# Farmadupe/vid_dup_finder_lib

Measured on AMD Instinct MI355X. Metric: hash-pairs/sec all-pairs Hamming (search(), tolerance 0.35) [+ frames/sec DCT-hash in 'summary.hash_summary'], higher is better.
Workload: dtype fp4 e2m1 ({0,1}) x fp4 -> f32 accumulate (exact half-integers < 2^11)

## Files before the change

vid_dup_finder_lib_amd/csrc/api.cpp:

```cpp
#include <algorithm>
#include <chrono>
#include <cmath>
#include <cstdio>
#include <cstdlib>
#include <cstring>
#include <memory>
#include <numeric>

#include "host_sort.h"
#include "vdf_ctx.h"
#include "window_class_layout.h"

namespace {
thread_local std::string g_create_error;
inline double now_ms() { return std::chrono::duration<double, std::milli>(std::chrono::steady_clock::now().time_since_epoch()).count(); }
}

vdf_ctx::~vdf_ctx()
{
    if (!subs.empty() || !workers.empty()) vdf_impl::destroy_multi(this);
    if (copy_pool) vdf_impl::destroy_copy_pool(this);
    for (auto &kv : axis_tables) {
        kv.second->start.release(); kv.second->size.release(); kv.second->w.release();
        delete kv.second;
    }
    for (auto &kv : mfma_tables) {
        kv.second->operand.release(); kv.second->bias.release(); kv.second->meta.release();
        delete kv.second;
    }
    for (auto &kv : box_tables) {
        kv.second->blob.release(); kv.second->entries.release();
        delete kv.second;
    }
    DevBuf *all[] = {&row_lo, &row_hi, &tile_lo, &tile_hi, &tile_first, &tile_count, &tile_offset, &counters,
                     &hits, &perm, &matched, &exp_cols, &exp_rows, &pop_cols, &pop_rows, &cand, &group_cmin, &group_offset, &group_blocks, &up_hashes,
                     &up_dur, &up_ref_hashes, &up_ref_dur, &small, &frames, &frames2, &out_hashes, &out_hashes2, &out_dc,
                     &out_dc2, &cos_table, &crops, &crop_desc, &crop_tables, &crop_desc2, &crop_tables2, &crop_work, &sort_scratch, &sort_scratch_pub, &hits2, &hit_bitmaps, &bitmap_gather,
                     &out_zero, &out_zero2, &up_zero, &variant_hashes, &align_plan, &align_scratch, &align_up, &seed_bitmap, &seed_plan, &seed_out, &seed_classes};
    for (DevBuf *b : all) b->release();
    for (PinBuf &b : pin) b.release();
    for (PinBuf &b : pin_out) b.release();
    pin_small.release();
    pin_ctrl.release();
    pin_crops.release();
    pin_desc.release();
    host_hits.buf.release();
    if (ev0) (void)hipEventDestroy(ev0);
    if (ev1) (void)hipEventDestroy(ev1);
    if (ev_mid) (void)hipEventDestroy(ev_mid);
    if (ev_wait) (void)hipEventDestroy(ev_wait);
    for (hipEvent_t e : ev_copy) if (e) (void)hipEventDestroy(e);
    for (hipEvent_t e : ev_done) if (e) (void)hipEventDestroy(e);
    if (copy_stream) (void)hipStreamDestroy(copy_stream);
    if (stream) (void)hipStreamDestroy(stream);
}

namespace vdf_impl {

void set_create_error(const std::string &msg) { g_create_error = msg; }

int fail(vdf_ctx *ctx, int code, const std::string &msg)
{
    if (ctx) ctx->err = msg;
    return code;
}

int fail_hip(vdf_ctx *ctx, hipError_t e, const char *what)
{
    std::string msg = std::string(what) + ": " + hipGetErrorString(e);
    (void)hipGetLastError();
    return fail(ctx, e == hipErrorOutOfMemory ? VDF_E_OOM : VDF_E_HIP, msg);
}

bool is_sorted_u32(const uint32_t *d, size_t n)
{
    for (size_t i = 1; i < n; i++)
        if (d[i] < d[i - 1]) return false;
    return true;
}

constexpr size_t kPinSmallBytes = 4u << 20;
constexpr uint64_t kDeviceSortHits = 1u << 17;
constexpr uint32_t kRefsMinWorkgroups = 2048;
constexpr uint64_t kSpecSortHits = 1u << 14;
constexpr uint64_t kFilterHits = 1u << 16;

int search_core(vdf_ctx *ctx, int mode, const uint64_t *d_col_hashes, const uint32_t *d_col_dur, size_t n_cols,
                const uint64_t *d_row_hashes, const uint32_t *d_row_dur, const uint32_t *d_row_perm, size_t n_rows,
                uint32_t tol_int, uint32_t shard_index, uint32_t shard_count, uint32_t row_begin, uint32_t row_end,
                const uint32_t *d_matched, uint32_t row_index_base, vdf_hit *hits, uint64_t capacity,
                uint64_t *n_hits_out, uint32_t *overflow_row_out, hipStream_t stream, bool replay_only, vdf_ctx::HostHits *staging,
                ShardExchange *fx)
{
    *n_hits_out = 0;
    *overflow_row_out = 0xFFFFFFFFu;
    if (n_rows == 0 || n_cols == 0) return VDF_OK;
    if (n_rows >= 0xFFFFFFFFull || n_cols >= 0xFFFFFFFFull) return fail(ctx, VDF_E_INVAL, "more than 2^32-1 hashes");
    if (shard_count == 0 || shard_index >= shard_count) return fail(ctx, VDF_E_INVAL, "bad shard index/count");
    VDF_HIP(ctx, hipSetDevice(ctx->device));
    const double t_enter = now_ms();

    vdf::SearchLaunch L{};
    const bool mfma = ctx->search_backend == 1;
    L.tile_rows = mfma ? (mode == 1 ? ctx->mfma_refs_rows : ctx->mfma_self_rows) : ctx->tile_rows;
    L.chunk_cols = mfma ? ctx->mfma_chunk_cols : ctx->chunk_cols;
    L.n_row_tiles = (uint32_t)((n_rows + L.tile_rows - 1) / L.tile_rows);
    if (mfma && L.chunk_cols == 0) {
        L.chunk_cols = 65536;
        while (L.chunk_cols > 4096 && (uint64_t)L.n_row_tiles * ((n_cols + L.chunk_cols - 1) / L.chunk_cols) < ctx->mfma_min_wgs) L.chunk_cols /= 2;
    }
    while ((uint64_t)L.n_row_tiles * ((n_cols + L.chunk_cols - 1) / L.chunk_cols) >= 0x40000000ull && L.chunk_cols < (1u << 22))
        L.chunk_cols *= 2;
    const size_t padded_rows = (size_t)L.n_row_tiles * L.tile_rows;
    VDF_HIP(ctx, ctx->row_lo.reserve(padded_rows * 4));
    VDF_HIP(ctx, ctx->row_hi.reserve(padded_rows * 4));
    VDF_HIP(ctx, ctx->tile_lo.reserve((size_t)L.n_row_tiles * 4));
    VDF_HIP(ctx, ctx->tile_hi.reserve((size_t)L.n_row_tiles * 4));
    VDF_HIP(ctx, ctx->tile_first.reserve((size_t)L.n_row_tiles * 4));
    VDF_HIP(ctx, ctx->tile_count.reserve((size_t)L.n_row_tiles * 4));
    VDF_HIP(ctx, ctx->tile_offset.reserve(((size_t)L.n_row_tiles + 1) * 4));
    VDF_HIP(ctx, ctx->counters.reserve(64));
    const uint64_t dev_cap = std::max<uint64_t>(capacity, 1);
    VDF_HIP(ctx, ctx->hits.reserve(dev_cap * sizeof(vdf_hit)));

    L.row_hashes = reinterpret_cast<const uint32_t *>(d_row_hashes);
    L.row_perm = d_row_perm;
    L.n_rows = (uint32_t)n_rows;
    L.row_index_base = row_index_base;
    L.col_hashes = reinterpret_cast<const uint32_t *>(d_col_hashes);
    L.n_cols = (uint32_t)n_cols;
    L.row_lo = ctx->row_lo.as<uint32_t>();
    L.row_hi = ctx->row_hi.as<uint32_t>();
    L.tile_lo = ctx->tile_lo.as<uint32_t>();
    L.tile_hi = ctx->tile_hi.as<uint32_t>();
    L.tile_first = ctx->tile_first.as<uint32_t>();
    L.tile_count = ctx->tile_count.as<uint32_t>();
    L.tile_offset = ctx->tile_offset.as<uint32_t>();
    L.tol = tol_int;
    L.matched = d_matched;
    L.self_mode = (mode == 0);
    L.shard_index = shard_index;
    L.shard_count = shard_count;
    L.hits = ctx->hits.as<vdf_hit>();
    L.capacity = capacity;
    L.counters = ctx->counters.as<unsigned long long>();
    L.overflow_row = reinterpret_cast<uint32_t *>(ctx->counters.as<unsigned long long>() + 4);

    L.prune_step = 16;
    if (ctx->mfma_prune_step >= 0) {
        L.prune_step = ctx->mfma_prune_step;
    } else {
        for (int st = 6; st <= 14; st++) {
            const double bits = 64.0 * (st + 1);
            if (bits / 2 - 2.0 * std::sqrt(bits) >= (double)tol_int + 1) { L.prune_step = st; break; }
        }
    }
    if (mfma) L.prune_step = L.prune_step <= 6 ? 6 : L.prune_step <= 8 ? 8 : L.prune_step <= 10 ? 10 : L.prune_step <= 14 ? L.prune_step : 16;
    else L.prune_step = L.prune_step <= 6 ? 6 : L.prune_step <= 10 ? 10 : L.prune_step <= 12 ? 12 : 16;
    if (mfma) {
        L.group_size = std::min<uint32_t>(ctx->mfma_group, L.n_row_tiles);
        L.n_groups = (L.n_row_tiles + L.group_size - 1) / L.group_size;
        if (L.n_groups > 1024) return fail(ctx, VDF_E_INVAL, "too many row-tile groups");
        VDF_HIP(ctx, ctx->group_cmin.reserve((size_t)L.n_groups * 4));
        VDF_HIP(ctx, ctx->group_offset.reserve(((size_t)L.n_groups + 1) * 4));
        VDF_HIP(ctx, ctx->group_blocks.reserve((size_t)L.n_groups * 4));
        L.group_blocks = ctx->group_blocks.as<uint32_t>();
        L.group_cmin = ctx->group_cmin.as<uint32_t>();
        L.group_offset = ctx->group_offset.as<uint32_t>();
        const uint32_t k_steps = (uint32_t)(L.prune_step < 15 ? L.prune_step + 1 : 16);
        const uint32_t col_pad = (uint32_t)((n_cols + vdf::kMfmaRowPad - 1) / vdf::kMfmaRowPad * vdf::kMfmaRowPad) + vdf::kMfmaColPad;
        VDF_HIP(ctx, ctx->exp_cols.reserve((size_t)col_pad * 512));
        VDF_HIP(ctx, ctx->pop_cols.reserve((size_t)col_pad * 12));
        const ExpOwner want_owner{d_col_hashes, n_cols, k_steps, ctx->exp_cols.p};
        const bool reuse = ctx->pinned_db == d_col_hashes && ctx->pinned_n == n_cols && ctx->exp_owner == want_owner;
        if (!reuse) {
            ctx->exp_owner = ExpOwner{};
            VDF_HIP(ctx, vdf::launch_expand_fp4(L.col_hashes, (uint32_t)n_cols, col_pad, ctx->exp_cols.p, k_steps,
                                                ctx->pop_cols.as<float>(), stream));
            ctx->exp_owner = want_owner;
        }
        L.col_exp = ctx->exp_cols.p;
        L.col_pop3 = ctx->pop_cols.as<float>();
        L.col_pad = col_pad;
        if (d_row_hashes == d_col_hashes) {
            L.row_exp = ctx->exp_cols.p;
            L.row_pop3 = L.col_pop3;
            L.row_pad = col_pad;
        } else {
            const uint32_t row_pad = (uint32_t)((padded_rows + 127) / 128 * 128);
            VDF_HIP(ctx, ctx->exp_rows.reserve((size_t)row_pad * 512));
            VDF_HIP(ctx, ctx->pop_rows.reserve((size_t)row_pad * 12));
            VDF_HIP(ctx, vdf::launch_expand_fp4(L.row_hashes, (uint32_t)n_rows, row_pad, ctx->exp_rows.p, k_steps,
                                                ctx->pop_rows.as<float>(), stream));
            L.row_exp = ctx->exp_rows.p;
            L.row_pop3 = ctx->pop_rows.as<float>();
            L.row_pad = row_pad;
        }
    }
    const unsigned long long init[8] = {0, 0, 0, 0, 0xFFFFFFFFull, 0, 0, 0};
    const bool pin_ok = ctx->pin_small.reserve(kPinSmallBytes) && ctx->pin_small.pinned;
    uint64_t spec = std::min<uint64_t>(capacity, std::max<uint64_t>(ctx->hits_guess + ctx->hits_guess / 4 + 1024, 8192));
    if (!pin_ok || spec * sizeof(vdf_hit) > kPinSmallBytes) spec = 0;
    const bool spec_sort = spec && ctx->hits_guess >= kSpecSortHits;
    if (spec_sort) VDF_HIP(ctx, hipMemsetAsync(ctx->hits.p, 0xFF, (size_t)spec * sizeof(vdf_hit), stream));
    const bool adapt_refs = mode == 1 && mfma && ctx->mfma_chunk_cols == 0;
    if (adapt_refs && ctx->refs_hint_cols == n_cols && ctx->refs_hint_rows == n_rows && ctx->refs_hint_chunk) L.chunk_cols = ctx->refs_hint_chunk;
    if (!ctx->pin_ctrl.reserve(256)) return fail(ctx, VDF_E_OOM, "pinned staging");
    unsigned long long *pre = ctx->pin_ctrl.as<unsigned long long>() + 8;
    uint32_t total_tiles = 0;
    unsigned long long unsorted = 0, admitted = 0;
    for (int pass = 0;; pass++) {
        VDF_HIP(ctx, hipMemcpyAsync(ctx->counters.p, init, sizeof init, hipMemcpyHostToDevice, stream));
        VDF_HIP(ctx, vdf::launch_windows_tiles(mode, d_col_dur, (uint32_t)n_cols, d_row_dur, d_row_perm, (uint32_t)n_rows,
                                               row_begin, row_end, shard_index, shard_count, L, stream));
        VDF_HIP(ctx, hipMemcpyAsync(pre, L.counters, 64, hipMemcpyDeviceToHost, stream));
        VDF_HIP(ctx, hipMemcpyAsync(pre + 8, mfma ? L.group_offset + L.n_groups : L.tile_offset + L.n_row_tiles, 4,
                                    hipMemcpyDeviceToHost, stream));
        VDF_HIP(ctx, hipMemcpyAsync(pre + 9, L.tile_offset + L.n_row_tiles, 4, hipMemcpyDeviceToHost, stream));
        VDF_HIP(ctx, hipStreamSynchronize(stream));
        total_tiles = *reinterpret_cast<const uint32_t *>(pre + 8);
        const uint32_t busy_tiles = *reinterpret_cast<const uint32_t *>(pre + 9);
        unsorted = pre[5];
        admitted = pre[2];
        if (!adapt_refs || pass > 0 || unsorted || busy_tiles == 0 || busy_tiles >= kRefsMinWorkgroups || L.chunk_cols <= 4096) break;
        uint64_t est = busy_tiles;
        while (L.chunk_cols > 4096 && est < kRefsMinWorkgroups) { L.chunk_cols /= 2; est *= 2; }
    }
    if (adapt_refs) { ctx->refs_hint_cols = n_cols; ctx->refs_hint_rows = n_rows; ctx->refs_hint_chunk = L.chunk_cols; }
    if (unsorted) return fail(ctx, VDF_E_INVAL, "durations are not ascending: pass the arrays in Search::sort order");
    if (total_tiles >= 0x7FFFFFFFu) return fail(ctx, VDF_E_INVAL, "tile count exceeds the grid limit");
    if (mfma) {
        const uint64_t want = ((uint64_t)((double)admitted * 6e-6) + (uint64_t)total_tiles * 8 * 8 + std::max<uint64_t>(capacity, 1ull << 20)) * ctx->cand_scale;
        L.cand_capacity = (uint32_t)std::min<uint64_t>(want, 0x40000000ull);
        if (ctx->cand_capacity_override)
            L.cand_capacity = (uint32_t)std::min<uint64_t>((uint64_t)ctx->cand_capacity_override * ctx->cand_scale, 0x40000000ull);
        const void *before = ctx->cand.p;
        VDF_HIP(ctx, ctx->cand.reserve((size_t)L.cand_capacity * 16));
        if (ctx->cand.p != before) ctx->cand_dirty = SIZE_MAX;
        const size_t slots = ctx->cand.cap / 16;
        const size_t fill = (ctx->cand_dirty == SIZE_MAX ? slots : std::min<size_t>(slots, ctx->cand_dirty)) * 16;
        if (fill) VDF_HIP(ctx, hipMemsetAsync(ctx->cand.p, 0xFF, fill, stream));
        ctx->cand_dirty = L.cand_capacity;
        L.cand = ctx->cand.p;
        L.cand_head = ctx->counters.as<unsigned long long>() + 6;
    }

    ctx->timing.prep_ms += (float)(now_ms() - t_enter);
    VDF_HIP(ctx, hipEventRecord(ctx->ev0, stream));
    if (mfma) {
        VDF_HIP(ctx, vdf::launch_hamming_tiles_mfma2(L, total_tiles, stream));
        VDF_HIP(ctx, hipEventRecord(ctx->ev_mid, stream));
        if (total_tiles) VDF_HIP(ctx, vdf::launch_resolve_candidates(L, stream));
    } else {
        VDF_HIP(ctx, vdf::launch_hamming_tiles(L, total_tiles, stream));
        VDF_HIP(ctx, hipEventRecord(ctx->ev_mid, stream));
    }
    VDF_HIP(ctx, hipEventRecord(ctx->ev1, stream));
    if (!ctx->pin_ctrl.reserve(256)) return fail(ctx, VDF_E_OOM, "pinned staging");
    unsigned long long *fin = ctx->pin_ctrl.as<unsigned long long>();
    VDF_HIP(ctx, hipMemcpyAsync(fin, ctx->counters.p, 64, hipMemcpyDeviceToHost, stream));
    unsigned row_bits = 1;
    while (row_bits < 32 && ((uint64_t)row_index_base + n_rows) >> row_bits) row_bits++;
    unsigned col_bits = 1;
    while (col_bits < 32 && ((uint64_t)n_cols >> col_bits)) col_bits++;
    if (spec_sort) {
        VDF_HIP(ctx, ctx->sort_scratch.reserve(vdf::sort_hits_scratch_bytes((size_t)spec)));
        VDF_HIP(ctx, vdf::launch_sort_hits(ctx->hits.as<vdf_hit>(), (size_t)spec, row_bits, ctx->sort_scratch.p, ctx->sort_scratch.cap, stream, col_bits));
    }
    if (spec) VDF_HIP(ctx, hipMemcpyAsync(ctx->pin_small.p, ctx->hits.p, (size_t)spec * sizeof(vdf_hit), hipMemcpyDeviceToHost, stream));
    VDF_HIP(ctx, hipStreamSynchronize(stream));
    const double t_synced = now_ms();
    float ms = 0.f, ms_stream = 0.f;
    VDF_HIP(ctx, hipEventElapsedTime(&ms, ctx->ev0, ctx->ev1));
// ... 3799 lines not shown
```

vid_dup_finder_lib_amd/csrc/hamming.hip:

```cpp
#include <algorithm>

#include "vdf_internal.h"

namespace vdf {

constexpr uint32_t kMaxBlocksPerLaunch = 4u << 20;

typedef const __attribute__((address_space(4))) uint32_t *const_u32_ptr;

__device__ __forceinline__ uint32_t sat_u32(double x)
{
    if (!(x == x)) return 0u;
    if (x <= 0.0) return 0u;
    if (x >= 4294967295.0) return 0xFFFFFFFFu;
    return (uint32_t)x;
}

__device__ __forceinline__ uint32_t partition_point_lt(const uint32_t *__restrict__ d, uint32_t n, uint32_t v)
{
    uint32_t lo = 0, hi = n;
    while (lo < hi) {
        uint32_t mid = lo + ((hi - lo) >> 1);
        if (d[mid] < v) lo = mid + 1; else hi = mid;
    }
    return lo;
}
__device__ __forceinline__ uint32_t partition_point_le(const uint32_t *__restrict__ d, uint32_t n, uint32_t v)
{
    uint32_t lo = 0, hi = n;
    while (lo < hi) {
        uint32_t mid = lo + ((hi - lo) >> 1);
        if (d[mid] <= v) lo = mid + 1; else hi = mid;
    }
    return lo;
}

__device__ __forceinline__ uint32_t wave_min(uint32_t v)
{
#pragma unroll
    for (int o = 32; o > 0; o >>= 1) v = min(v, (uint32_t)__shfl_xor((int)v, o, 64));
    return v;
}
__device__ __forceinline__ uint32_t wave_max(uint32_t v)
{
#pragma unroll
    for (int o = 32; o > 0; o >>= 1) v = max(v, (uint32_t)__shfl_xor((int)v, o, 64));
    return v;
}

__device__ __forceinline__ void wave_append_hits(bool hit, uint32_t row, uint32_t col, vdf_hit *__restrict__ hits,
                                                 unsigned long long capacity, unsigned long long *__restrict__ counters,
                                                 uint32_t *__restrict__ overflow_row)
{
    const unsigned long long bal = __builtin_amdgcn_ballot_w64(hit);
    if (bal == 0ull) return;
    const int leader = __builtin_ctzll(bal);
    unsigned long long base = 0;
    if ((int)(threadIdx.x & 63) == leader) base = atomicAdd(&counters[0], (unsigned long long)__builtin_popcountll(bal));
    base = ((unsigned long long)(uint32_t)__shfl((int)(base >> 32), leader, 64) << 32) | (uint32_t)__shfl((int)(uint32_t)base, leader, 64);
    if (hit) {
        const unsigned long long at = base + __builtin_amdgcn_mbcnt_hi((uint32_t)(bal >> 32), __builtin_amdgcn_mbcnt_lo((uint32_t)bal, 0u));
        if (at < capacity) {
            vdf_hit hp; hp.row = row; hp.col = col;
            hits[at] = hp;
        } else {
            atomicMin(overflow_row, row);
        }
    }
}

__global__ __launch_bounds__(256) void windows_tiles_kernel(
    int mode, const uint32_t *__restrict__ col_dur, uint32_t n_cols, const uint32_t *__restrict__ row_dur,
    const uint32_t *__restrict__ row_perm, uint32_t n_rows, uint32_t row_begin, uint32_t row_end, uint32_t shard_index,
    uint32_t shard_count, uint32_t tile_rows, uint32_t chunk_cols, uint32_t *__restrict__ row_lo,
    uint32_t *__restrict__ row_hi, uint32_t *__restrict__ tile_lo, uint32_t *__restrict__ tile_hi,
    uint32_t *__restrict__ tile_first, uint32_t *__restrict__ tile_count, unsigned long long *__restrict__ counters)
{
    __shared__ uint32_t s_min[4], s_max[4];
    __shared__ unsigned long long s_pairs[4];
    const uint32_t t = blockIdx.x;
    const bool mine = (t % shard_count) == shard_index;
    uint32_t mn = 0xFFFFFFFFu, mx = 0u;
    unsigned long long pairs = 0;
    for (uint32_t q = threadIdx.x; q < tile_rows; q += 256) {
// ... 156 lines not shown
#pragma unroll
            for (int q = 0; q < 8; q++) {
                const uint4 v = rp[q];
                rw[k][4 * q + 0] = v.x; rw[k][4 * q + 1] = v.y; rw[k][4 * q + 2] = v.z; rw[k][4 * q + 3] = v.w;
            }
            if (self_mode && matched && ((matched[src >> 5] >> (src & 31)) & 1u)) { lo = 0; hi = 0; }
        } else {
#pragma unroll
            for (int q = 0; q < 32; q++) rw[k][q] = 0u;
            lo = 0; hi = 0;
        }
        rlo[k] = lo; rhi[k] = hi; rid[k] = row_index_base + src;
    }

    const_u32_ptr cols = (const_u32_ptr)(uintptr_t)col_hashes;
    uint32_t n_early = 0;
    for (uint32_t c = c_begin; c < c_end; ++c) {
        const_u32_ptr cp = cols + (size_t)c * 32;
        uint32_t d[R];
#pragma unroll
        for (int k = 0; k < R; k++) d[k] = 0u;
#pragma unroll
        for (int w = 0; w < (CHKW < 32 ? CHKW : 32); ++w) {
            const uint32_t cw = cp[w];
#pragma unroll
            for (int k = 0; k < R; k++) d[k] += __builtin_popcount(rw[k][w] ^ cw);
        }
        uint32_t m = d[0];
#pragma unroll
        for (int k = 1; k < R; k++) m = min(m, d[k]);
        if (CHKW < 32) {
            if (__builtin_amdgcn_ballot_w64(m <= tol) == 0ull) { n_early += 1; continue; }
#pragma unroll
            for (int w = CHKW; w < 32; ++w) {
                const uint32_t cw = cp[w];
#pragma unroll
                for (int k = 0; k < R; k++) d[k] += __builtin_popcount(rw[k][w] ^ cw);
            }
            m = d[0];
#pragma unroll
            for (int k = 1; k < R; k++) m = min(m, d[k]);
        }
        if (__builtin_amdgcn_ballot_w64(m <= tol) != 0ull) {
            bool col_ok = true;
            if (matched) col_ok = ((((const_u32_ptr)(uintptr_t)matched)[c >> 5] >> (c & 31)) & 1u) == 0u;
            if (col_ok) {
#pragma unroll
                for (int k = 0; k < R; k++)
                    wave_append_hits(d[k] <= tol && c >= rlo[k] && c < rhi[k], rid[k], c, hits, capacity, counters, overflow_row);
            }
        }
    }
    if (threadIdx.x == 0) atomicAdd(&counters[1], (unsigned long long)(c_end - c_begin) * TILE_ROWS);
    if (CHKW < 32 && lane == 0 && n_early) atomicAdd(&counters[3], (unsigned long long)n_early * (64u * R));
}

typedef int v8i __attribute__((ext_vector_type(8)));
typedef int v4i __attribute__((ext_vector_type(4)));
typedef float v16f __attribute__((ext_vector_type(16)));

__global__ __launch_bounds__(256) void expand_fp4_kernel(const uint32_t *__restrict__ packed, uint32_t n,
                                                        uint32_t n_pad, uint4 *__restrict__ expanded,
                                                        uint32_t k_steps, float *__restrict__ pop,
                                                        float *__restrict__ popk, float *__restrict__ popkT)
{
    for (size_t idx = (size_t)blockIdx.x * 256 + threadIdx.x; idx < (size_t)n_pad * 32;
         idx += (size_t)gridDim.x * 256) {
    const uint32_t hsh = (uint32_t)(idx >> 5), dw = (uint32_t)idx & 31u;
    uint4 out = {0u, 0u, 0u, 0u};
    uint32_t w = 0;
    if (hsh < n) {
        w = packed[idx];
        uint32_t o[4];
#pragma unroll
        for (int j = 0; j < 4; j++) {
            uint32_t x = (w >> (8 * j)) & 0xFFu;
            x = (x | (x << 12)) & 0x000F000Fu;
            x = (x | (x << 6)) & 0x03030303u;
            x = (x | (x << 3)) & 0x11111111u;
            o[j] = x << 1;
        }
        out = make_uint4(o[0], o[1], o[2], o[3]);
    }
    expanded[idx] = out;
    if (pop) {
        uint32_t pc = (uint32_t)__builtin_popcount(w), pk = (dw & 15u) < k_steps ? pc : 0u;
#pragma unroll
        for (int o = 16; o > 0; o >>= 1) { pc += (uint32_t)__shfl_xor((int)pc, o, 32); pk += (uint32_t)__shfl_xor((int)pk, o, 32); }
        if (dw == 0) {
            pop[hsh] = (float)pc;
            popk[hsh] = (float)pk;
            popkT[(size_t)(hsh >> 7) * 128 + (hsh & 31u) * 4 + ((hsh >> 5) & 3u)] = (float)pk;
        }
    }
    }
}

template <int N>
struct IntC { static constexpr int value = N; };
template <int I, int N, class F>
__device__ __forceinline__ void static_for(F &&f)
{
    if constexpr (I < N) {
        f(IntC<I>{});
        static_for<I + 1, N>(f);
    }
}

constexpr uint32_t rowterm_row_of_lane(uint32_t l) { return (l & 3u) + 8u * ((l & 15u) >> 2) + 4u * (l >> 5); }
constexpr bool rowterm_map_matches_c_layout()
{
    for (uint32_t g = 0; g < 2; g++)
        for (uint32_t half = 0; half < 2; half++)
            for (uint32_t r = 0; r < 16; r++)
                if (rowterm_row_of_lane(32u * g + 16u * half + r) != (r & 3u) + 8u * (r >> 2) + 4u * g) return false;
    return true;
}
static_assert(rowterm_map_matches_c_layout(), "row-term lanes do not match the MFMA C layout");

struct CandEntry {
    uint32_t row_base;
    uint32_t col;
    uint32_t mask;
    uint32_t pad;
};

__global__ __launch_bounds__(256) void resolve_candidates_kernel(
    const CandEntry *__restrict__ cand, const unsigned long long *__restrict__ cand_head, uint32_t cand_capacity,
    const uint32_t *__restrict__ row_hashes, const uint32_t *__restrict__ row_perm, uint32_t n_rows, uint32_t row_index_base,
    const uint32_t *__restrict__ col_hashes, uint32_t n_cols, const uint32_t *__restrict__ row_lo,
    const uint32_t *__restrict__ row_hi, uint32_t tol, const uint32_t *__restrict__ matched, int self_mode,
    vdf_hit *__restrict__ hits, unsigned long long capacity, unsigned long long *__restrict__ counters,
    uint32_t *__restrict__ overflow_row)
{
    const uint32_t n = (uint32_t)min(*cand_head, (unsigned long long)cand_capacity);
    const uint32_t lane = threadIdx.x & 63, wave = threadIdx.x >> 6;
    constexpr uint32_t kStage = 512;
    __shared__ vdf_hit s_stage[4][kStage];
    uint32_t staged = 0;
    auto flush = [&]() {
        if (staged == 0) return;
        __builtin_amdgcn_fence(__ATOMIC_ACQ_REL, "wavefront");
        __builtin_amdgcn_wave_barrier();
        unsigned long long base = 0;
        if (lane == 0) base = atomicAdd(&counters[0], (unsigned long long)staged);
        base = ((unsigned long long)(uint32_t)__builtin_amdgcn_readfirstlane((int)(base >> 32)) << 32) |
               (uint32_t)__builtin_amdgcn_readfirstlane((int)(uint32_t)base);
        for (uint32_t k = lane; k < staged; k += 64) {
            const vdf_hit hp = s_stage[wave][k];
            if (base + k < capacity) hits[base + k] = hp;
            else atomicMin(overflow_row, hp.row);
        }
        __builtin_amdgcn_fence(__ATOMIC_ACQ_REL, "wavefront");
        __builtin_amdgcn_wave_barrier();
        staged = 0;
    };
    for (uint32_t e0 = blockIdx.x * 256 + (threadIdx.x & ~63u); e0 < n; e0 += gridDim.x * 256) {
        const uint32_t e = e0 + lane;
        CandEntry ce;
        ce.row_base = 0xFFFFFFFFu; ce.col = 0; ce.mask = 0; ce.pad = 0;
        if (e < n) ce = cand[e];
        uint32_t m = ce.mask;
        if (ce.row_base == 0xFFFFFFFFu || ce.col >= n_cols) m = 0;
        if (m && matched && ((matched[ce.col >> 5] >> (ce.col & 31)) & 1u)) m = 0;
        uint4 cw[8];
        if (m) {
            const uint4 *cp = reinterpret_cast<const uint4 *>(col_hashes + (size_t)ce.col * 32);
#pragma unroll
            for (int q = 0; q < 8; q++) cw[q] = cp[q];
        }
        while (__builtin_amdgcn_ballot_w64(m != 0u) != 0ull) {
            bool hit = false;
            uint32_t src = 0;
            if (m) {
                const uint32_t r = (uint32_t)__builtin_ctz(m);
                m &= m - 1;
                const uint32_t p = ce.row_base + (r & 3) + 8 * (r >> 2);
                if (p < n_rows) {
                    const uint32_t lo = row_lo[p], hi = row_hi[p];
                    if (ce.col >= lo && ce.col < hi) {
                        src = row_perm ? row_perm[p] : p;
                        if (!(self_mode && matched && ((matched[src >> 5] >> (src & 31)) & 1u))) {
                            const uint4 *rp = reinterpret_cast<const uint4 *>(row_hashes + (size_t)src * 32);
                            uint32_t d = 0;
#pragma unroll
                            for (int q = 0; q < 8; q++) {
                                const uint4 v = rp[q];
                                d += __builtin_popcount(v.x ^ cw[q].x) + __builtin_popcount(v.y ^ cw[q].y) +
                                     __builtin_popcount(v.z ^ cw[q].z) + __builtin_popcount(v.w ^ cw[q].w);
                            }
                            hit = d <= tol;
                        }
                    }
                }
            }
            const unsigned long long bal = __builtin_amdgcn_ballot_w64(hit);
            if (bal == 0ull) continue;
            const uint32_t cnt = (uint32_t)__builtin_popcountll(bal);
            if (staged + cnt > kStage) flush();
            if (hit) {
                vdf_hit hp; hp.row = row_index_base + src; hp.col = ce.col;
                s_stage[wave][staged + __builtin_amdgcn_mbcnt_hi((uint32_t)(bal >> 32), __builtin_amdgcn_mbcnt_lo((uint32_t)bal, 0u))] = hp;
            }
            staged += cnt;
        }
    }
    flush();
}

template <int CHK, int WAVES>
__global__ __launch_bounds__(64 * WAVES, 2) void hamming_mfma2_kernel(
    const uint4 *__restrict__ row_exp, const uint32_t *__restrict__ row_perm, uint32_t n_rows,
    uint32_t row_index_base, const uint4 *__restrict__ col_exp, const uint32_t *__restrict__ row_lo,
    const uint32_t *__restrict__ row_hi, const uint32_t *__restrict__ tile_lo, const uint32_t *__restrict__ tile_hi,
    const uint32_t *__restrict__ tile_first, const uint32_t *__restrict__ tile_count,
    const uint32_t *__restrict__ group_offset, const uint32_t *__restrict__ group_cmin, uint32_t n_groups,
    uint32_t group_size, uint32_t shard_index, uint32_t shard_count, uint32_t n_row_tiles, uint32_t chunk_cols,
    uint32_t tol, const uint32_t *__restrict__ matched, int self_mode, vdf_hit *__restrict__ hits,
    unsigned long long capacity, unsigned long long *__restrict__ counters, uint32_t *__restrict__ overflow_row,
    uint32_t block_base, const float *__restrict__ row_pop3, uint32_t row_pad, const float *__restrict__ col_pop3,
    uint32_t col_pad, CandEntry *__restrict__ cand, uint32_t cand_capacity, unsigned long long *__restrict__ cand_head)
{
    constexpr int K = CHK < 15 ? CHK + 1 : 16;
    constexpr bool kRowcLds = K > 13;
    constexpr bool kLock = K >= 9 && K <= 13;
    constexpr int PL = 2, NBL = PL + 1;
    constexpr int kLoadAt = 10;
    constexpr uint32_t kSub = WAVES >= 8 ? 4 : 2;
    constexpr uint32_t kColStep = 32 * kSub;
    constexpr int NBLK = 2 * (int)kSub;
    constexpr int NM = NBLK * K;
    constexpr int P = (K == 16 && WAVES >= 8) ? 2 : 4, NB = P + 1;
    constexpr uint32_t kTileRows = 64 * WAVES;
    constexpr int kDmaPerWave = (int)(kColStep * 32 / (64 * WAVES));
    constexpr int kDmaEvery = NM / kDmaPerWave;
    static_assert(kDmaEvery >= 2, "stage too short for its DMA pieces");
    constexpr int kTestAt = 2;
    static_assert(K >= kTestAt + 4, "block too short to hide the previous block's test");
    static_assert(!kLock || (kLoadAt >= kTestAt + 8 && 2 * K >= kLoadAt + 8), "pair too short for two tests and the re-load of two sets");
    const uint32_t bid = blockIdx.x + block_base;
    __shared__ __attribute__((aligned(16))) uint4 s_b0[kColStep * 32];
    __shared__ __attribute__((aligned(16))) uint4 s_b1[kColStep * 32];
    const uint32_t tid = threadIdx.x, lane = tid & 63, g = lane >> 5, c31 = lane & 31;
    const uint32_t wave = (uint32_t)__builtin_amdgcn_readfirstlane((int)(tid >> 6));

    const_u32_ptr goff = (const_u32_ptr)(uintptr_t)group_offset;
    uint32_t gl = 0, gh = n_groups;
    while (gh - gl > 1) {
        const uint32_t mid = (gl + gh) >> 1;
        if (goff[mid] <= bid) gl = mid; else gh = mid;
    }
    const uint32_t idx = bid - goff[gl];
    const uint32_t per_group = (group_size + shard_count - 1) / shard_count;
    const uint32_t g0 = gl * group_size;
    const uint32_t t0 = g0 + (shard_index + shard_count - g0 % shard_count) % shard_count;
    const uint32_t t = t0 + (idx % per_group) * shard_count;
    const uint32_t chunk = ((const_u32_ptr)(uintptr_t)group_cmin)[gl] + idx / per_group;
    if (t >= n_row_tiles || t >= g0 + group_size) return;
    {
        const uint32_t f = ((const_u32_ptr)(uintptr_t)tile_first)[t], cnt = ((const_u32_ptr)(uintptr_t)tile_count)[t];
        if (chunk < f || chunk >= f + cnt) return;
    }
    const uint32_t t_lo = ((const_u32_ptr)(uintptr_t)tile_lo)[t];
    const uint32_t t_hi = ((const_u32_ptr)(uintptr_t)tile_hi)[t];
    const uint32_t c_begin = max(chunk * chunk_cols, t_lo);
    const uint32_t c_end = min((chunk + 1) * chunk_cols, t_hi);
    if (c_begin >= c_end) return;

    const float tol_f = (float)min(tol, 1024u);
    const float *row_popk = row_pop3 + row_pad;
    const float *col_popkT = col_pop3 + 2 * (size_t)col_pad;
    const uint32_t row0 = t * kTileRows + wave * 64;
    v4i a[2][K];
    const float4 *s_rc = nullptr;
    v16f rowc[2];
    float rowv[2] = {0.f, 0.f};
    uint32_t live[2];
#pragma unroll
    for (int rt = 0; rt < 2; rt++) {
        live[rt] = 0;
        const uint32_t p = row0 + 32 * rt + c31;
        uint32_t src = p;
        if (p < n_rows && row_perm) src = row_perm[p];
        const uint4 *rp = row_exp + (size_t)src * 32 + 16 * g;
#pragma unroll
        for (int s = 0; s < K; s++) {
            const uint4 v = rp[s];
            a[rt][s] = (v4i){(int)v.x, (int)v.y, (int)v.z, (int)v.w};
        }
        if constexpr (kLock) {
            const uint32_t pr = row0 + 32 * rt + rowterm_row_of_lane(lane);
            const uint32_t sr = (pr < n_rows && row_perm) ? row_perm[pr] : pr;
            rowv[rt] = -0.5f * row_popk[sr];
            live[rt] = (uint32_t)(__builtin_amdgcn_ballot_w64(row_hi[pr] > row_lo[pr]) >> (32 * g)) & 0xFFFFu;
        } else {
#pragma unroll
            for (int r = 0; r < 16; r++) {
                const uint32_t pr = row0 + 32 * rt + (r & 3) + 8 * (r >> 2) + 4 * g;
                const uint32_t sr = (pr < n_rows && row_perm) ? row_perm[pr] : pr;
                rowc[rt][r] = -0.5f * row_popk[sr];
                if (row_hi[pr] > row_lo[pr]) live[rt] |= 1u << r;
            }
        }
    }
    if constexpr (kRowcLds) {
        __shared__ __attribute__((aligned(16))) float4 s_rowc[WAVES * 2 * 2 * 4];
        float4 *mine = s_rowc + ((size_t)wave * 2 * 2 + g) * 4;
        if (c31 == 0) {
#pragma unroll
            for (int rt = 0; rt < 2; rt++)
#pragma unroll
                for (int q = 0; q < 4; q++)
                    mine[rt * 2 * 4 + q] = float4{rowc[rt][4 * q], rowc[rt][4 * q + 1], rowc[rt][4 * q + 2], rowc[rt][4 * q + 3]};
        }
        s_rc = mine;
    }
    const uint32_t cb0 = c_begin & ~(kColStep - 1);
    constexpr uint32_t kColsPerRound = 2 * WAVES;
    constexpr int kOffsets = 32 / kColsPerRound;
    static_assert(kOffsets >= 1 && (kOffsets & (kOffsets - 1)) == 0, "piece addressing");
    const uint32_t c0 = 2 * wave + g;
    uint32_t lane_off[kOffsets];
#pragma unroll
    for (int j = 0; j < kOffsets; j++) lane_off[j] = c0 * 512u + ((((lane & 31) ^ c0) << 4) ^ (16u * kColsPerRound * j));
    auto stage_rsrc = [&](uint32_t cb) __attribute__((always_inline)) {
        return __builtin_amdgcn_make_buffer_rsrc(
            const_cast<char *>(reinterpret_cast<const char *>(col_exp) + (size_t)cb * 512), 0, kColStep * 512u, 0x00020000);
    };
    auto load_piece = [&](__amdgpu_buffer_rsrc_t rs, uint4 *dst, int i) __attribute__((always_inline)) {
        auto *lds = (__attribute__((address_space(3))) void *)&dst[64 * WAVES * i + 64 * wave];
        const int voff = (int)lane_off[i & (kOffsets - 1)], soff = (int)(512u * kColsPerRound * (uint32_t)i);
        __builtin_amdgcn_raw_ptr_buffer_load_lds(rs, lds, 16, voff, soff, 0, 0);
    };
    auto load_thr = [&](uint32_t cb, float (&out)[kSub]) __attribute__((always_inline)) {
        const float *q = col_popkT + (size_t)(cb >> 7) * 128 + c31 * 4 + ((cb >> 5) & 3u);
        if constexpr (kSub == 4) {
            const float4 v = *reinterpret_cast<const float4 *>(q);
            out[0] = v.x; out[1] = v.y; out[2] = v.z; out[3] = v.w;
        } else {
            const float2 v = *reinterpret_cast<const float2 *>(q);
            out[0] = v.x; out[1] = v.y;
        }
    };

    v16f acc[2] = {v16f{}, v16f{}};
    if constexpr (kRowcLds) acc[0] = rowc[0];
    v16f acc4[4] = {v16f{}, v16f{}, v16f{}, v16f{}};
    auto load_rowterm = [&](v16f &c, float v, auto rc) __attribute__((always_inline)) {
        constexpr int r = decltype(rc)::value;
        c[r] = __int_as_float(__builtin_amdgcn_update_dpp(__float_as_int(c[r]), __float_as_int(v), 0x150 + r, 0xF, 0xF, false));
    };
    if constexpr (kLock) {
        static_for<0, 16>([&](auto rc) __attribute__((always_inline)) { load_rowterm(acc4[0], rowv[0], rc); load_rowterm(acc4[1], rowv[1], rc); });
    }
    uint32_t n_early = 0;
    float thr[kSub], thr_next[kSub];

    constexpr uint32_t kCandChunk = 8, kCandChunkMax = 512;
    uint32_t q_chunk = kCandChunk, q_taken = 0;
    unsigned long long q_next = 0, q_end = 0;
    auto emit = [&](const v16f &c, float thrv, uint32_t live_rows, uint32_t rows_first, uint32_t col_first) __attribute__((always_inline)) {
        uint32_t mask = 0;
#pragma unroll
        for (int r = 0; r < 16; r++) mask |= (c[r] >= thrv) ? (1u << r) : 0u;
        mask &= live_rows;
        const uint32_t j = col_first + c31;
        if (j < c_begin || j >= c_end) mask = 0;
        const unsigned long long bal = __builtin_amdgcn_ballot_w64(mask != 0u);
        if (bal == 0ull) return;
        const uint32_t need = (uint32_t)__builtin_popcountll(bal);
        if (q_next + need > q_end) {
            if (q_taken >= 2) q_chunk = min(2u * q_chunk, kCandChunkMax);
            q_taken++;
            const uint32_t take = max((need + kCandChunk - 1) / kCandChunk * kCandChunk, q_chunk);
            unsigned long long base = 0;
            if (lane == 0) base = atomicAdd(cand_head, (unsigned long long)take);
            q_next = ((unsigned long long)(uint32_t)__builtin_amdgcn_readfirstlane((int)(base >> 32)) << 32) |
                     (uint32_t)__builtin_amdgcn_readfirstlane((int)(uint32_t)base);
            q_end = q_next + take;
        }
        const unsigned long long slot = q_next + __builtin_amdgcn_mbcnt_hi((uint32_t)(bal >> 32), __builtin_amdgcn_mbcnt_lo((uint32_t)bal, 0u));
        if (mask != 0u) {
            if (slot < cand_capacity) {
                CandEntry ce; ce.row_base = rows_first + 4 * g; ce.col = j; ce.mask = mask; ce.pad = 0;
                *reinterpret_cast<uint4 *>(&cand[slot]) = *reinterpret_cast<const uint4 *>(&ce);
            } else {
                const uint32_t p = rows_first + 4 * g + (uint32_t)(__builtin_ctz(mask) & 3) + 8 * (uint32_t)(__builtin_ctz(mask) >> 2);
                if (p < n_rows) atomicMin(overflow_row, row_index_base + (row_perm ? row_perm[p] : p));
            }
        }
        q_next += need;
    };

    auto end_stage = [&](uint32_t cb, uint32_t flags) __attribute__((always_inline)) {
        uint32_t valid = 0;
#pragma unroll
        for (uint32_t sub = 0; sub < kSub; sub++)
            if (cb + 32u * sub < c_end) valid |= 3u << (2 * sub);
        flags &= valid;
        n_early += (uint32_t)__builtin_popcount(valid & ~flags);
        asm volatile("s_waitcnt vmcnt(0)" ::: "memory");
        __syncthreads();
#pragma unroll
        for (uint32_t sub = 0; sub < kSub; sub++) thr[sub] = 0.5f * (thr_next[sub] - tol_f);
    };

    auto run_stage = [&](uint32_t cb, const uint4 *cur, uint4 *nxt) __attribute__((always_inline)) {
        const uint32_t cb_next = cb + kColStep < c_end ? cb + kColStep : cb;
        const __amdgpu_buffer_rsrc_t rs_next = stage_rsrc(cb_next);
        load_thr(cb_next, thr_next);
        uint32_t flags = 0;
        uint4 fq[NB];
        auto frag = [&](int i) __attribute__((always_inline)) {
            const uint32_t sub = (uint32_t)((i / K) >> 1), s = (uint32_t)(i % K);
            return cur[((32u * sub + c31) << 5) | ((s + 16u * g) ^ c31)];
        };
#pragma unroll
        for (int i = 0; i < P; i++) fq[i] = frag(i);
        __builtin_amdgcn_sched_barrier(0);
        float m0 = 0.f, m1 = 0.f, m2 = 0.f, m3 = 0.f, m4 = 0.f, m5 = 0.f;
        static_for<0, NM>([&](auto ic) __attribute__((always_inline)) {
            constexpr int i = decltype(ic)::value;
            constexpr int blk = i / K, s = i % K, rt = blk & 1;
            const uint4 bv = fq[i % NB];
            const v8i b = {(int)bv.x, (int)bv.y, (int)bv.z, (int)bv.w, 0, 0, 0, 0};
            const v8i ar = {a[rt][s].x, a[rt][s].y, a[rt][s].z, a[rt][s].w, 0, 0, 0, 0};
            if constexpr (s == 0 && !kRowcLds) acc[rt] = __builtin_amdgcn_mfma_scale_f32_32x32x64_f8f6f4(ar, b, rowc[rt], 4, 4, 0, 0, 0, 0);
            else acc[rt] = __builtin_amdgcn_mfma_scale_f32_32x32x64_f8f6f4(ar, b, acc[rt], 4, 4, 0, 0, 0, 0);
            if constexpr (i + P < NM) fq[(i + P) % NB] = frag(i + P);
            if constexpr ((i % kDmaEvery) == 1 && (i / kDmaEvery) < kDmaPerWave) load_piece(rs_next, nxt, i / kDmaEvery);
            if constexpr (blk >= 1) {
                const v16f &c = acc[rt ^ 1];
                if constexpr (s == kTestAt) {
                    m0 = fmaxf(fmaxf(c[0], c[1]), c[2]); m1 = fmaxf(fmaxf(c[3], c[4]), c[5]); m2 = fmaxf(fmaxf(c[6], c[7]), c[8]);
                } else if constexpr (s == kTestAt + 1) {
                    m3 = fmaxf(fmaxf(c[9], c[10]), c[11]); m4 = fmaxf(fmaxf(c[12], c[13]), c[14]);
                } else if constexpr (s == kTestAt + 2) {
                    m5 = fmaxf(fmaxf(m0, m1), m2); m3 = fmaxf(fmaxf(m3, m4), c[15]);
                } else if constexpr (s == kTestAt + 3) {
                    if (__builtin_amdgcn_ballot_w64(fmaxf(m5, m3) >= thr[(blk - 1) >> 1]) != 0ull) {
                        flags |= 1u << (blk - 1);
                        emit(c, thr[(blk - 1) >> 1], live[rt ^ 1], row0 + 32u * (uint32_t)(rt ^ 1), cb + 32u * (uint32_t)((blk - 1) >> 1));
                    }
                }
            }
            if constexpr (kRowcLds && s >= kTestAt + 4 && s < kTestAt + 8) {
                constexpr int q = s - (kTestAt + 4);
                const float4 v = s_rc[((rt ^ 1) * 2) * 4 + q];
                acc[rt ^ 1][4 * q + 0] = v.x; acc[rt ^ 1][4 * q + 1] = v.y; acc[rt ^ 1][4 * q + 2] = v.z; acc[rt ^ 1][4 * q + 3] = v.w;
            }
            __builtin_amdgcn_sched_barrier(0);
        });
        {
            const v16f &c = acc[(NBLK - 1) & 1];
            m0 = fmaxf(fmaxf(c[0], c[1]), c[2]); m1 = fmaxf(fmaxf(c[3], c[4]), c[5]); m2 = fmaxf(fmaxf(c[6], c[7]), c[8]);
            m3 = fmaxf(fmaxf(c[9], c[10]), c[11]); m4 = fmaxf(fmaxf(c[12], c[13]), c[14]);
            const float pm = fmaxf(fmaxf(fmaxf(m0, m1), m2), fmaxf(fmaxf(m3, m4), c[15]));
            if (__builtin_amdgcn_ballot_w64(pm >= thr[kSub - 1]) != 0ull) {
                flags |= 1u << (NBLK - 1);
                emit(c, thr[kSub - 1], live[(NBLK - 1) & 1], row0 + 32u * (uint32_t)((NBLK - 1) & 1), cb + 32u * (kSub - 1));
            }
        }
        end_stage(cb, flags);
    };

    auto run_stage_lock = [&](uint32_t cb, const uint4 *cur, uint4 *nxt) __attribute__((always_inline)) {
        const uint32_t cb_next = cb + kColStep < c_end ? cb + kColStep : cb;
        const __amdgpu_buffer_rsrc_t rs_next = stage_rsrc(cb_next);
        load_thr(cb_next, thr_next);
        uint32_t flags = 0;
        uint4 fq[NBL];
        constexpr int NF = (int)kSub * K;
        auto frag = [&](int f) __attribute__((always_inline)) {
            const uint32_t sub = (uint32_t)(f / K), s = (uint32_t)(f % K);
            return cur[((32u * sub + c31) << 5) | ((s + 16u * g) ^ c31)];
        };
#pragma unroll
        for (int f = 0; f < PL; f++) fq[f] = frag(f);
        __builtin_amdgcn_sched_barrier(0);
        float m0 = 0.f, m1 = 0.f, m2 = 0.f, m3 = 0.f, m4 = 0.f, m5 = 0.f;
        static_for<0, NM>([&](auto ic) __attribute__((always_inline)) {
            constexpr int i = decltype(ic)::value;
            constexpr int p = i / (2 * K), j = i % (2 * K), s = j >> 1, rt = j & 1, f = p * K + s;
            constexpr int mine = 2 * (p & 1) + rt, other = 2 * ((p & 1) ^ 1);
            const uint4 bv = fq[f % NBL];
            const v8i b = {(int)bv.x, (int)bv.y, (int)bv.z, (int)bv.w, 0, 0, 0, 0};
            const v8i ar = {a[rt][s].x, a[rt][s].y, a[rt][s].z, a[rt][s].w, 0, 0, 0, 0};
            acc4[mine] = __builtin_amdgcn_mfma_scale_f32_32x32x64_f8f6f4(ar, b, acc4[mine], 4, 4, 0, 0, 0, 0);
            if constexpr (rt == 0 && f + PL < NF) fq[(f + PL) % NBL] = frag(f + PL);
            if constexpr ((i % kDmaEvery) == 1 && (i / kDmaEvery) < kDmaPerWave) load_piece(rs_next, nxt, i / kDmaEvery);
            if constexpr (p >= 1 && j >= kTestAt && j < kTestAt + 8) {
                constexpr int trt = (j - kTestAt) >> 2, q = (j - kTestAt) & 3;
                const v16f &c = acc4[other + trt];
                if constexpr (q == 0) {
                    m0 = fmaxf(fmaxf(c[0], c[1]), c[2]); m1 = fmaxf(fmaxf(c[3], c[4]), c[5]); m2 = fmaxf(fmaxf(c[6], c[7]), c[8]);
                } else if constexpr (q == 1) {
                    m3 = fmaxf(fmaxf(c[9], c[10]), c[11]); m4 = fmaxf(fmaxf(c[12], c[13]), c[14]);
                } else if constexpr (q == 2) {
                    m5 = fmaxf(fmaxf(m0, m1), m2); m3 = fmaxf(fmaxf(m3, m4), c[15]);
                } else {
                    if (__builtin_amdgcn_ballot_w64(fmaxf(m5, m3) >= thr[p - 1]) != 0ull) {
                        flags |= 1u << (2 * (p - 1) + trt);
                        emit(c, thr[p - 1], live[trt], row0 + 32u * (uint32_t)trt, cb + 32u * (uint32_t)(p - 1));
                    }
                }
            }
            if constexpr (j >= kLoadAt && j < kLoadAt + 8) {
                constexpr int lrt = (j - kLoadAt) >> 2, q = (j - kLoadAt) & 3;
                static_for<4 * q, 4 * q + 4>([&](auto rc) __attribute__((always_inline)) { load_rowterm(acc4[other + lrt], rowv[lrt], rc); });
            }
            __builtin_amdgcn_sched_barrier(0);
        });
        static_for<0, 2>([&](auto rtc) __attribute__((always_inline)) {
            constexpr int rt = decltype(rtc)::value;
            const v16f &c = acc4[2 * (((int)kSub - 1) & 1) + rt];
            m0 = fmaxf(fmaxf(c[0], c[1]), c[2]); m1 = fmaxf(fmaxf(c[3], c[4]), c[5]); m2 = fmaxf(fmaxf(c[6], c[7]), c[8]);
            m3 = fmaxf(fmaxf(c[9], c[10]), c[11]); m4 = fmaxf(fmaxf(c[12], c[13]), c[14]);
            const float pm = fmaxf(fmaxf(fmaxf(m0, m1), m2), fmaxf(fmaxf(m3, m4), c[15]));
            if (__builtin_amdgcn_ballot_w64(pm >= thr[kSub - 1]) != 0ull) {
                flags |= 1u << (2 * ((int)kSub - 1) + rt);
                emit(c, thr[kSub - 1], live[rt], row0 + 32u * (uint32_t)rt, cb + 32u * (kSub - 1));
            }
        });
        end_stage(cb, flags);
    };
    auto stage =[&](uint32_t cb, const uint4 *cur, uint4 *nxt) __attribute__((always_inline)) {
        if constexpr (kLock) run_stage_lock(cb, cur, nxt);
        else run_stage(cb, cur, nxt);
    };

#pragma unroll
    for (int i = 0; i < kDmaPerWave; i++) load_piece(stage_rsrc(cb0), s_b0, i);
    load_thr(cb0, thr_next);
#pragma unroll
    for (int rt = 0; rt < 2; rt++)
#pragma unroll
        for (int s = 0; s < K; s++) asm volatile("" ::"v"(a[rt][s]));
    asm volatile("s_waitcnt vmcnt(0)" ::: "memory");
    __syncthreads();
#pragma unroll
    for (uint32_t sub = 0; sub < kSub; sub++) thr[sub] = 0.5f * (thr_next[sub] - tol_f);
    for (uint32_t cb = cb0; cb < c_end; cb += 2 * kColStep) {
        stage(cb, s_b0, s_b1);
        if (cb + kColStep >= c_end) break;
        stage(cb + kColStep, s_b1, s_b0);
    }
    if (tid == 0) atomicAdd(&counters[1], (unsigned long long)(c_end - c_begin) * kTileRows);
    if (CHK < 15 && lane == 0 && n_early) atomicAdd(&counters[3], (unsigned long long)n_early * (32u * 32u));
}

__global__ __launch_bounds__(256) void hits_mark_incoming_kernel(const vdf_hit *__restrict__ hits, unsigned long long n,
                                                                 uint32_t *__restrict__ has_in)
{
    for (size_t i = (size_t)blockIdx.x * 256 + threadIdx.x; i < n; i += (size_t)gridDim.x * 256) {
        const uint32_t j = hits[i].col;
        if (!((has_in[j >> 5] >> (j & 31)) & 1u)) atomicOr(&has_in[j >> 5], 1u << (j & 31));
    }
}
// ... 231 lines not shown
```

Baseline: 4807 billion.

## Store only the used K-steps per hash in a compact padded fp4 image

Replaces the fixed 512-byte-per-hash expanded fp4 layout with a compact image that stores only the 2*K chunks actually consumed by the pruned MFMA passes, plus one pad chunk that makes the stride odd. This cuts global-to-LDS DMA traffic and LDS footprint per stage when K<16. The odd stride replaces the XOR swizzle for avoiding LDS bank conflicts, and fragment addresses fold into compile-time offsets. Risks include changed bank-conflict behaviour, uneven DMA piece distribution across waves, and a different LDS size that may shift occupancy.

```diff
diff --git a/vid_dup_finder_lib_amd/csrc/api.cpp b/vid_dup_finder_lib_amd/csrc/api.cpp
--- a/vid_dup_finder_lib_amd/csrc/api.cpp
+++ b/vid_dup_finder_lib_amd/csrc/api.cpp
@@ -7,6 +7,7 @@
 #include <memory>
 #include <numeric>
 
+#include "fp4_image_layout.h"
 #include "host_sort.h"
 #include "vdf_ctx.h"
 #include "window_class_layout.h"
@@ -169,7 +170,7 @@
         L.group_offset = ctx->group_offset.as<uint32_t>();
         const uint32_t k_steps = (uint32_t)(L.prune_step < 15 ? L.prune_step + 1 : 16);
         const uint32_t col_pad = (uint32_t)((n_cols + vdf::kMfmaRowPad - 1) / vdf::kMfmaRowPad * vdf::kMfmaRowPad) + vdf::kMfmaColPad;
-        VDF_HIP(ctx, ctx->exp_cols.reserve((size_t)col_pad * 512));
+        VDF_HIP(ctx, ctx->exp_cols.reserve(vdf::fp4_image_bytes(col_pad, k_steps)));
         VDF_HIP(ctx, ctx->pop_cols.reserve((size_t)col_pad * 12));
         const ExpOwner want_owner{d_col_hashes, n_cols, k_steps, ctx->exp_cols.p};
         const bool reuse = ctx->pinned_db == d_col_hashes && ctx->pinned_n == n_cols && ctx->exp_owner == want_owner;
@@ -188,7 +189,7 @@
             L.row_pad = col_pad;
         } else {
             const uint32_t row_pad = (uint32_t)((padded_rows + 127) / 128 * 128);
-            VDF_HIP(ctx, ctx->exp_rows.reserve((size_t)row_pad * 512));
+            VDF_HIP(ctx, ctx->exp_rows.reserve(vdf::fp4_image_bytes(row_pad, k_steps)));
             VDF_HIP(ctx, ctx->pop_rows.reserve((size_t)row_pad * 12));
             VDF_HIP(ctx, vdf::launch_expand_fp4(L.row_hashes, (uint32_t)n_rows, row_pad, ctx->exp_rows.p, k_steps,
                                                 ctx->pop_rows.as<float>(), stream));
diff --git a/vid_dup_finder_lib_amd/csrc/fp4_image_layout.h b/vid_dup_finder_lib_amd/csrc/fp4_image_layout.h
--- /dev/null
+++ b/vid_dup_finder_lib_amd/csrc/fp4_image_layout.h
@@ -0,0 +1,65 @@
+#pragma once
+#include <stddef.h>
+#include <stdint.h>
+
+#if defined(__HIPCC__) || defined(__CUDACC__)
+#define VDF_FP4_IMAGE_HD __host__ __device__
+#else
+#define VDF_FP4_IMAGE_HD
+#endif
+
+namespace vdf {
+
+constexpr uint32_t kFp4ChunkBytes = 16;
+constexpr uint32_t kFp4PieceBytes = 1024;
+constexpr uint32_t kFp4NoChunk = 0xFFFFFFFFu;
+constexpr uint32_t kFp4PadDword = 0xFFFFFFFEu;
+
+VDF_FP4_IMAGE_HD constexpr uint32_t fp4_image_stride(uint32_t k) { return 2u * k + 1u; }
+VDF_FP4_IMAGE_HD constexpr uint32_t fp4_image_stride_bytes(uint32_t k) { return kFp4ChunkBytes * fp4_image_stride(k); }
+VDF_FP4_IMAGE_HD constexpr size_t fp4_image_bytes(size_t n, uint32_t k) { return n * (size_t)fp4_image_stride_bytes(k); }
+VDF_FP4_IMAGE_HD constexpr size_t fp4_image_hash_offset(size_t h, uint32_t k) { return h * (size_t)fp4_image_stride_bytes(k); }
+
+VDF_FP4_IMAGE_HD constexpr uint32_t fp4_image_chunk(uint32_t dword, uint32_t k)
+{
+    return (dword & 15u) < k ? (dword >> 4) * k + (dword & 15u) : kFp4NoChunk;
+}
+VDF_FP4_IMAGE_HD constexpr uint32_t fp4_image_dword(uint32_t chunk, uint32_t k)
+{
+    return chunk < k ? chunk : chunk < 2u * k ? 16u + (chunk - k) : kFp4PadDword;
+}
+VDF_FP4_IMAGE_HD constexpr uint32_t fp4_image_pad_chunk(uint32_t k) { return 2u * k; }
+
+VDF_FP4_IMAGE_HD constexpr size_t fp4_image_row_chunk(size_t src, uint32_t s, uint32_t g, uint32_t k)
+{
+    return src * fp4_image_stride(k) + (size_t)k * g + s;
+}
+VDF_FP4_IMAGE_HD constexpr uint32_t fp4_image_stage_chunk(uint32_t col, uint32_t s, uint32_t g, uint32_t k)
+{
+    return col * fp4_image_stride(k) + k * g + s;
+}
+
+VDF_FP4_IMAGE_HD constexpr uint32_t fp4_image_stage_chunks(uint32_t col_step, uint32_t k) { return col_step * fp4_image_stride(k); }
+VDF_FP4_IMAGE_HD constexpr uint32_t fp4_image_stage_bytes(uint32_t col_step, uint32_t k) { return kFp4ChunkBytes * fp4_image_stage_chunks(col_step, k); }
+VDF_FP4_IMAGE_HD constexpr uint32_t fp4_image_pieces(uint32_t col_step, uint32_t k) { return fp4_image_stage_bytes(col_step, k) / kFp4PieceBytes; }
+VDF_FP4_IMAGE_HD constexpr uint32_t fp4_image_rounds(uint32_t col_step, uint32_t k, uint32_t waves)
+{
+    return (fp4_image_pieces(col_step, k) + waves - 1u) / waves;
+}
+VDF_FP4_IMAGE_HD constexpr uint32_t fp4_image_piece(uint32_t round, uint32_t wave, uint32_t waves) { return round * waves + wave; }
+VDF_FP4_IMAGE_HD constexpr bool fp4_image_wave_has_piece(uint32_t round, uint32_t wave, uint32_t waves, uint32_t col_step, uint32_t k)
+{
+    return fp4_image_piece(round, wave, waves) < fp4_image_pieces(col_step, k);
+}
+VDF_FP4_IMAGE_HD constexpr uint32_t fp4_image_piece_slot(uint32_t piece) { return piece * (kFp4PieceBytes / kFp4ChunkBytes); }
+VDF_FP4_IMAGE_HD constexpr uint32_t fp4_image_piece_offset(uint32_t piece) { return piece * kFp4PieceBytes; }
+
+VDF_FP4_IMAGE_HD constexpr uint32_t fp4_image_lane_group(uint32_t lane)
+{
+    const uint32_t l = lane & 31u;
+    const bool first = l < 4u || (l >= 12u && l < 16u) || (l >= 20u && l < 28u);
+    return 2u * (lane >> 5) + (first ? 0u : 1u);
+}
+VDF_FP4_IMAGE_HD constexpr uint32_t fp4_image_bank_slot(uint32_t chunk) { return chunk & 15u; }
+
+}
diff --git a/vid_dup_finder_lib_amd/csrc/hamming.hip b/vid_dup_finder_lib_amd/csrc/hamming.hip
--- a/vid_dup_finder_lib_amd/csrc/hamming.hip
+++ b/vid_dup_finder_lib_amd/csrc/hamming.hip
@@ -1,5 +1,6 @@
 #include <algorithm>
 
+#include "fp4_image_layout.h"
 #include "vdf_internal.h"
 
 namespace vdf {
@@ -322,7 +323,10 @@
         }
         out = make_uint4(o[0], o[1], o[2], o[3]);
     }
-    expanded[idx] = out;
+    uint4 *img = expanded + (size_t)hsh * fp4_image_stride(k_steps);
+    const uint32_t chunk = fp4_image_chunk(dw, k_steps);
+    if (chunk != kFp4NoChunk) img[chunk] = out;
+    if (dw == 0) img[fp4_image_pad_chunk(k_steps)] = make_uint4(0u, 0u, 0u, 0u);
     if (pop) {
         uint32_t pc = (uint32_t)__builtin_popcount(w), pk = (dw & 15u) < k_steps ? pc : 0u;
 #pragma unroll
@@ -472,15 +476,18 @@
     constexpr int NM = NBLK * K;
     constexpr int P = (K == 16 && WAVES >= 8) ? 2 : 4, NB = P + 1;
     constexpr uint32_t kTileRows = 64 * WAVES;
-    constexpr int kDmaPerWave = (int)(kColStep * 32 / (64 * WAVES));
+    constexpr uint32_t kStageChunks = fp4_image_stage_chunks(kColStep, K);
+    constexpr uint32_t kPieces = fp4_image_pieces(kColStep, K);
+    constexpr int kDmaPerWave = (int)fp4_image_rounds(kColStep, K, WAVES);
     constexpr int kDmaEvery = NM / kDmaPerWave;
+    static_assert(kPieces * kFp4PieceBytes == kStageChunks * kFp4ChunkBytes, "a stage is a whole number of pieces");
     static_assert(kDmaEvery >= 2, "stage too short for its DMA pieces");
     constexpr int kTestAt = 2;
     static_assert(K >= kTestAt + 4, "block too short to hide the previous block's test");
     static_assert(!kLock || (kLoadAt >= kTestAt + 8 && 2 * K >= kLoadAt + 8), "pair too short for two tests and the re-load of two sets");
     const uint32_t bid = blockIdx.x + block_base;
-    __shared__ __attribute__((aligned(16))) uint4 s_b0[kColStep * 32];
-    __shared__ __attribute__((aligned(16))) uint4 s_b1[kColStep * 32];
+    __shared__ __attribute__((aligned(16))) uint4 s_b0[kStageChunks];
+    __shared__ __attribute__((aligned(16))) uint4 s_b1[kStageChunks];
     const uint32_t tid = threadIdx.x, lane = tid & 63, g = lane >> 5, c31 = lane & 31;
     const uint32_t wave = (uint32_t)__builtin_amdgcn_readfirstlane((int)(tid >> 6));
 
@@ -522,7 +529,7 @@
         const uint32_t p = row0 + 32 * rt + c31;
         uint32_t src = p;
         if (p < n_rows && row_perm) src = row_perm[p];
-        const uint4 *rp = row_exp + (size_t)src * 32 + 16 * g;
+        const uint4 *rp = row_exp + fp4_image_row_chunk(src, 0, g, K);
 #pragma unroll
         for (int s = 0; s < K; s++) {
             const uint4 v = rp[s];
@@ -556,21 +563,20 @@
         s_rc = mine;
     }
     const uint32_t cb0 = c_begin & ~(kColStep - 1);
-    constexpr uint32_t kColsPerRound = 2 * WAVES;
-    constexpr int kOffsets = 32 / kColsPerRound;
-    static_assert(kOffsets >= 1 && (kOffsets & (kOffsets - 1)) == 0, "piece addressing");
-    const uint32_t c0 = 2 * wave + g;
-    uint32_t lane_off[kOffsets];
-#pragma unroll
-    for (int j = 0; j < kOffsets; j++) lane_off[j] = c0 * 512u + ((((lane & 31) ^ c0) << 4) ^ (16u * kColsPerRound * j));
+    const uint32_t frag_base = fp4_image_stage_chunk(c31, 0, g, K);
+    static_assert(fp4_image_stage_chunk(kColStep - 32, K - 1, 0, K) * kFp4ChunkBytes < 65536, "the compile-time part of a fragment address fits the instruction's offset field");
+    const uint32_t lane_off = fp4_image_piece_offset(wave) + lane * kFp4ChunkBytes;
     auto stage_rsrc = [&](uint32_t cb) __attribute__((always_inline)) {
         return __builtin_amdgcn_make_buffer_rsrc(
-            const_cast<char *>(reinterpret_cast<const char *>(col_exp) + (size_t)cb * 512), 0, kColStep * 512u, 0x00020000);
+            const_cast<char *>(reinterpret_cast<const char *>(col_exp) + fp4_image_hash_offset(cb, K)), 0,
+            fp4_image_stage_bytes(kColStep, K), 0x00020000);
     };
     auto load_piece = [&](__amdgpu_buffer_rsrc_t rs, uint4 *dst, int i) __attribute__((always_inline)) {
-        auto *lds = (__attribute__((address_space(3))) void *)&dst[64 * WAVES * i + 64 * wave];
-        const int voff = (int)lane_off[i & (kOffsets - 1)], soff = (int)(512u * kColsPerRound * (uint32_t)i);
-        __builtin_amdgcn_raw_ptr_buffer_load_lds(rs, lds, 16, voff, soff, 0, 0);
+        if ((uint32_t)(i + 1) * WAVES <= kPieces || fp4_image_wave_has_piece((uint32_t)i, wave, WAVES, kColStep, K)) {
+            auto *lds = (__attribute__((address_space(3))) void *)&dst[fp4_image_piece_slot(fp4_image_piece((uint32_t)i, wave, WAVES))];
+            const int soff = (int)fp4_image_piece_offset(fp4_image_piece((uint32_t)i, 0, WAVES));
+            __builtin_amdgcn_raw_ptr_buffer_load_lds(rs, lds, 16, (int)lane_off, soff, 0, 0);
+        }
     };
     auto load_thr = [&](uint32_t cb, float (&out)[kSub]) __attribute__((always_inline)) {
         const float *q = col_popkT + (size_t)(cb >> 7) * 128 + c31 * 4 + ((cb >> 5) & 3u);
@@ -651,9 +657,10 @@
         load_thr(cb_next, thr_next);
         uint32_t flags = 0;
         uint4 fq[NB];
+        const uint4 *cur_lane = cur + frag_base;
         auto frag = [&](int i) __attribute__((always_inline)) {
             const uint32_t sub = (uint32_t)((i / K) >> 1), s = (uint32_t)(i % K);
-            return cur[((32u * sub + c31) << 5) | ((s + 16u * g) ^ c31)];
+            return cur_lane[fp4_image_stage_chunk(32u * sub, s, 0, K)];
         };
 #pragma unroll
         for (int i = 0; i < P; i++) fq[i] = frag(i);
@@ -710,10 +717,11 @@
         load_thr(cb_next, thr_next);
         uint32_t flags = 0;
         uint4 fq[NBL];
+        const uint4 *cur_lane = cur + frag_base;
         constexpr int NF = (int)kSub * K;
         auto frag = [&](int f) __attribute__((always_inline)) {
             const uint32_t sub = (uint32_t)(f / K), s = (uint32_t)(f % K);
-            return cur[((32u * sub + c31) << 5) | ((s + 16u * g) ^ c31)];
+            return cur_lane[fp4_image_stage_chunk(32u * sub, s, 0, K)];
         };
 #pragma unroll
         for (int f = 0; f < PL; f++) fq[f] = frag(f);
```

After: 4817 billion, median of 6. No clear change (+0.2%).
